# WhenMelancholy/ray-tracing-in-cuda

Measured on AMD Instinct MI355X. Metric: Msamples/sec (WxHxspp), higher is better.
Workload: dtype f32; 1 GPU; RTIOW random-spheres scene (rt_scene_rtiow seed 7, 484 spheres), 1920x1080, 1024 spp, depth 50; spp_chunk=0, kernel_variant=0, render_seed=2023

## Files before the change

### include/rtmi.h

```cpp
#ifndef RTMI_H
#define RTMI_H

#include <stddef.h>
#include <stdint.h>

#ifdef __cplusplus
extern "C" {
#endif

#define RTMI_ABI_VERSION 3

typedef enum rt_status {
    RT_OK = 0,
    RT_ERR_ARG = 1,
    RT_ERR_IO = 2,
    RT_ERR_JSON = 3,
    RT_ERR_SCENE = 4,
    RT_ERR_HIP = 5,
    RT_ERR_LIMIT = 6
} rt_status;


typedef enum rt_prim_type {
    RT_PRIM_SPHERE = 0,
// ... 269 lines not shown
int rt_scene_table_image(const rt_scene *s, float *out, int cap_floats);


typedef struct rt_opts {
    uint64_t seed;
    int32_t device;
    int32_t tile_rows;
    int32_t tile_first;
    int32_t tile_stride;
    int32_t tile_rotate;
    int32_t spp_chunk;
    int32_t sample_first;
    int32_t sample_count;
    uint32_t variant;
} rt_opts;

typedef struct rt_stats {
    double kernel_ms;
    double upload_ms;
    int32_t launches;
    int32_t local_rows;
    uint64_t samples, queries, prim_tests, hits, misses;
    uint64_t scatter[4];
    uint64_t rng_draws;
    uint64_t cand_lanes, cand_waves;
    uint64_t clusters_visited;
    uint64_t wave_queries;
    uint64_t groups_visited;
    uint64_t lane_clusters;
    uint64_t lane_groups;
// ... 158 lines not shown
```

### include/rtmi.hpp

```cpp
#pragma once
#include <cmath>
#include <memory>
#include <stdexcept>
#include <string>
#include <vector>

#include "rtmi.h"

namespace rtmi {

struct vec3 {
    float e[3];
    vec3() : e{0, 0, 0} {}
    vec3(float x, float y, float z) : e{x, y, z} {}
    float x() const { return e[0]; }
    float y() const { return e[1]; }
    float z() const { return e[2]; }
};
using point3 = vec3;
using color = vec3;

struct error : std::runtime_error {
    int status;
    error(int st, const std::string &where)
// ... 359 lines not shown
    void set_projection(rt_projection_type type, float p0 = 0.0f, float p1 = 0.0f) {
        const float p[2] = {p0, p1};
        check(rt_scene_set_projection(s_, type, type == RT_PROJ_PERSPECTIVE ? nullptr : p), "set_projection");
    }
    rt_projection_type projection(float params[2] = nullptr) const {
        int type = 0;
        check(rt_scene_get_projection(s_, &type, params), "projection");
        return (rt_projection_type)type;
    }
    bool camera_ray(float s, float t, rt_ray &out, float lx = 0.0f, float ly = 0.0f) const {
        int valid = 0;
        check(rt_camera_ray(s_, s, t, lx, ly, &out, &valid), "camera_ray");
        return valid != 0;
    }

    std::vector<rt_hit> trace(const std::vector<rt_ray> &rays, const rt_opts *opts = nullptr) const {
        std::vector<rt_hit> out(rays.size());
        check(rt_trace_hip(s_, opts, RT_TRACE_CLOSEST, rays.data(), rays.size(), out.data(), nullptr), "trace");
        return out;
    }
    std::vector<uint8_t> occluded(const std::vector<rt_ray> &rays, const rt_opts *opts = nullptr) const {
        std::vector<uint8_t> out(rays.size());
        check(rt_trace_hip(s_, opts, RT_TRACE_OCCLUDED, rays.data(), rays.size(), out.data(), nullptr), "occluded");
        return out;
    }

    rt_scene_info info() const {
        rt_scene_info i;
        check(rt_scene_get_info(s_, &i), "info");
        return i;
// ... 166 lines not shown
```

### ray-tracing-in-cuda_amd/__init__.py

```python
from __future__ import annotations

import ctypes as C
import os

import numpy as np

try:
    import torch
except Exception:
    torch = None

_HERE = os.path.dirname(os.path.abspath(__file__))
_LIB_PATH = os.environ.get("RTMI_LIB") or os.path.join(_HERE, "librtmi.so")
if not os.path.exists(_LIB_PATH):
    raise ImportError(
        f"{_LIB_PATH} not found: build it with `make -C {_HERE}` (or __graft_entry__.build()); "
        "this package has no fallback implementation"
    )
_lib = C.CDLL(_LIB_PATH)

RT_OK = 0
FLAG_SKY_GRADIENT = 1
FLAG_DEFOCUS_BLUR = 2
PRIM_SPHERE, PRIM_XY_RECT, PRIM_XZ_RECT, PRIM_YZ_RECT, PRIM_CYLINDER, PRIM_TRIANGLE, PRIM_QUAD = range(7)
# ... 267 lines not shown
_sig("rt_scene_clear_moving_spheres", C.c_int, _p)
_sig("rt_moving_sphere_hit", C.c_int, _p, C.c_float, _f3, _f3, C.c_float, C.POINTER(C.c_float))
_sig("rt_shutter_time", C.c_float, C.c_uint64, C.c_uint32, C.c_uint32)
_sig("rt_scene_add_point_light", C.c_int, _p, _f3, _f3)
_sig("rt_scene_add_spot_light", C.c_int, _p, _f3, _f3, _f3, C.c_float, C.c_float)
_sig("rt_scene_add_distant_light", C.c_int, _p, _f3, _f3, C.c_float)
_sig("rt_scene_get_analytic_lights", C.c_int, _p, _p, C.c_int)
_sig("rt_scene_clear_analytic_lights", C.c_int, _p)
assert _lib.rt_struct_size(25) == ANALYTIC_LIGHT_DTYPE.itemsize == 48
_sig("rt_scene_set_nested_grid", C.c_int, _p, C.c_int)
_sig("rt_scene_get_nested_grid", C.c_int, _p)
_sig("rt_scene_nested_info", C.c_int, _p, C.POINTER(NestedInfo))
_sig("rt_render_hip_count", C.c_int, _p, C.POINTER(Opts), _p, C.POINTER(Stats))
_sig("rt_scene_table_info", C.c_int, _p, C.POINTER(TableInfo))
_sig("rt_scene_table_image", C.c_int, _p, _p, C.c_int)
_sig("rt_render_hip_accumulate", C.c_int, _p, C.POINTER(Opts), _p, _p, C.POINTER(Stats))
_sig("rt_acc_to_rgb", None, _p, _p, C.c_size_t)
_sig("rt_render_hip_adaptive", C.c_int, _p, C.POINTER(Opts), C.POINTER(Adaptive), _p, _p, C.POINTER(AdaptiveStats))
_sig("rt_render_hip_adaptive_device", C.c_int, _p, C.POINTER(Opts), C.POINTER(Adaptive), _p, _p, _p, C.POINTER(AdaptiveStats))
_sig("rt_shard_scatter_rows", C.c_int, _p, C.POINTER(Opts), _p, _p)
_sig("rt_write_ppm", C.c_int, C.c_char_p, _p, C.c_int, C.c_int, C.c_int)
_sig("rt_quantize_rgb8", C.c_int, _p, C.c_int, C.c_int, C.c_int, C.c_int, _p)
_sig("rt_write_png", C.c_int, C.c_char_p, _p, C.c_int, C.c_int, C.c_int, C.c_int)
_sig("rt_scene_output_file", C.c_char_p, _p)
_sig("rt_philox4x32_10", None, C.POINTER(C.c_uint32), C.POINTER(C.c_uint32), C.POINTER(C.c_uint32))
_sig("rt_aabb_hit", C.c_int, _f3, _f3, _f3, _f3, C.c_float, C.c_float)
_sig("rt_sample_stream", None, C.c_uint64, C.c_uint32, C.c_uint32, C.POINTER(C.c_uint32), C.c_int)
_sig("rt_render_hip_feature", C.c_int, _p, C.POINTER(Opts), C.c_int, _p, C.POINTER(Stats))
_sig("rt_render_hip_feature_device", C.c_int, _p, C.POINTER(Opts), C.c_int, _p, _p, C.POINTER(Stats))
_sig("rt_trace_hip", C.c_int, _p, C.POINTER(Opts), C.c_int, _p, C.c_size_t, _p, C.POINTER(Stats))
# ... 7 lines not shown
     C.POINTER(C.c_double))
_sig("rt_denoise_hip_device", C.c_int, C.c_int, C.c_int, _p, C.c_int, _p, _p, _p, _p, C.c_int, C.POINTER(Denoise), C.c_int, _p, _p,
     C.POINTER(C.c_double))
_sig("rt_display_hip", C.c_int, C.c_int, C.c_int, _p, C.c_int, _p, C.POINTER(Display), C.c_int, _p, _p, C.POINTER(DisplayStats))
_sig("rt_display_hip_device", C.c_int, C.c_int, C.c_int, _p, C.c_int, _p, C.POINTER(Display), C.c_int, _p, _p, _p,
     C.POINTER(DisplayStats))
_sig("rt_display_timing", C.c_int, C.POINTER(C.c_double), C.c_int)
_sig("rt_write_ppm_rgb8", C.c_int, C.c_char_p, _p, C.c_int, C.c_int)
_sig("rt_write_png_rgb8", C.c_int, C.c_char_p, _p, C.c_int, C.c_int)
_sig("rt_write_hdr", C.c_int, C.c_char_p, _p, C.c_int, C.c_int, C.c_int)
_sig("rt_write_pfm", C.c_int, C.c_char_p, _p, C.c_int, C.c_int, C.c_int)

C_SYMBOLS = [
    "rt_last_error", "rt_status_string", "rt_abi_version", "rt_struct_size", "rt_device_count", "rt_has_ablations", "rt_opts_default",
    "rt_scene_table_info", "rt_scene_table_image", "rt_variant_workgroup",
    "rt_scene_load_json", "rt_scene_parse_json", "rt_scene_rtiow", "rt_scene_to_json", "rt_scene_free",
    "rt_scene_new", "rt_scene_set_background", "rt_scene_set_camera", "rt_scene_add_solid_color",
    "rt_scene_add_checker", "rt_scene_add_lambertian", "rt_scene_add_metal", "rt_scene_add_dielectric",
    "rt_scene_add_rough_metal", "rt_scene_add_plastic", "rt_scene_add_rough_glass", "rt_scene_add_noise_texture", "rt_scene_get_noise",
    "rt_scene_set_bump", "rt_scene_get_bump", "rt_scene_set_normal_map", "rt_scene_get_normal_map",
    "rt_scene_add_image_texture_rgba", "rt_scene_get_image_alpha", "rt_scene_set_alpha", "rt_scene_get_alpha", "rt_scene_add_pbr", "rt_scene_set_pbr_map", "rt_scene_get_pbr_map",
    "rt_scene_add_diffuse_light", "rt_scene_add_sphere", "rt_scene_add_rect", "rt_scene_add_cylinder",
    "rt_scene_add_image_texture", "rt_scene_add_image_texture_file", "rt_scene_get_image", "rt_scene_add_triangle",
    "rt_scene_add_quad", "rt_scene_add_box", "rt_scene_add_obj", "rt_scene_add_triangle_normals", "rt_scene_add_obj_normals", "rt_set_mesh_normals_override",
    "rt_scene_override", "rt_scene_get_info", "rt_scene_get_camera", "rt_scene_get_prims",
    "rt_scene_get_materials", "rt_scene_get_textures", "rt_shard_rows", "rt_shard_global_row", "rt_shard_deal",
    "rt_render_hip_device", "rt_render_hip", "rt_render_hip_tiles", "rt_tiles_shutdown", "rt_shard_place_rows_device", "rt_render_hip_count", "rt_render_hip_accumulate", "rt_scene_set_russian_roulette",
    "rt_acc_to_rgb", "rt_shard_scatter_rows", "rt_write_ppm",
    "rt_quantize_rgb8", "rt_philox4x32_10", "rt_aabb_hit", "rt_sample_stream", "rt_write_png",
    "rt_scene_output_file", "rt_scene_rotate_cylinders", "rt_scene_set_output_file", "rt_scene_dna", "rt_scene_clone",
# ... 544 lines not shown
                                         C.byref(stats) if stats is not None else None), "rt_render_hip_device")

    def table_info(self) -> TableInfo:
        t = TableInfo()
        _check(_lib.rt_scene_table_info(self._h, C.byref(t)), "rt_scene_table_info")
        return t

    def table_image(self) -> np.ndarray:
        n = _lib.rt_scene_table_image(self._h, None, 0)
        if n < 0:
            raise RtmiError(-n, "rt_scene_table_image")
        out = np.empty(n, dtype=np.float32)
        _lib.rt_scene_table_image(self._h, out.ctypes.data_as(C.c_void_p), n)
        return out.reshape(-1, 4)

    def count(self, opts: Opts | None = None, want_image=False):
        opts = opts or Opts()
        st = Stats()
        out = None
        ptr = None
        if want_image:
            out = np.empty((self.shard_rows(opts), self.width, 3), dtype=np.float32)
            ptr = out.ctypes.data_as(C.c_void_p)
        _check(_lib.rt_render_hip_count(self._h, C.byref(opts), ptr, C.byref(st)), "rt_render_hip_count")
        return (st, out) if want_image else st

    def accumulate(self, acc: np.ndarray | None = None, opts: Opts | None = None, stats: Stats | None = None,
                   want_image=True):
        opts = opts or Opts()
        rows = self.shard_rows(opts)
# ... 232 lines not shown
```

### ray-tracing-in-cuda_amd/csrc/device_scene.h

```cpp
#pragma once
#include <stdint.h>

#ifndef RTMI_ABLATIONS
#define RTMI_ABLATIONS 1
#endif

#define RT_CLUSTER 8
#define RT_MAX_SPHERE_SLOTS (1LL << 28)

#define RT_LIGHT_STRIDE 7

#define RT_CYL_STRIDE 6
#define RT_TRI_STRIDE 5
#define RT_QUAD_STRIDE 5
static_assert(RT_QUAD_STRIDE == RT_TRI_STRIDE, "quads and triangles share one hot table");

#ifndef RT_GROUP
#define RT_GROUP 4
#endif

#ifndef RT_SLABS
#define RT_SLABS 16
#endif

// ... 14 lines not shown
    MK_LIGHT_IMAGE = 7,
    MK_MEDIUM = 8,
    MK_ROUGH_METAL = 9,
    MK_PLASTIC_SOLID = 10,
    MK_PLASTIC_CHECKER = 11,
    MK_PLASTIC_IMAGE = 12,
    MK_LAMBERT_NOISE = 13,
    MK_LIGHT_NOISE = 14,
    MK_PLASTIC_NOISE = 15,
    MK_ROUGH_GLASS = 16,
    MK_PBR = 18
};

#define RT_ITEM_PARAMS_AT 16
#define RT_TILE_LIST_AT 64
struct ItemParams {
    int32_t tiles_x, bands, num_items, sample_first, sample_count, spp_chunk, n_big, n_med, q_med, q_small;
    int32_t tile_rows, tile_first, tile_stride, local_rows;
    int32_t tile_rotate;
    int32_t n_list = 0;
};

#define RT_PFLAG_NORMAL_MAPS (1u << 16)
#define RT_PFLAG_PROJ_SHIFT 17
#define RT_ALPHA_MAX_PASSES 64

struct RenderParams {
    int32_t off_cam;
    float background[3];
    uint32_t flags;
// ... 67 lines not shown
```

### ray-tracing-in-cuda_amd/csrc/kernels.h

```cpp
#pragma once
#include <hip/hip_runtime.h>
#include <stddef.h>

#include "device_scene.h"

namespace rtmi {

enum KernelFamily {
    K_PLAIN,
    K_NEE,
    K_NESTED,
    K_FEATURE,
    K_ENV,
    K_MEDIA,
    K_MOTION,
    K_TRACE,
};

struct KernelKey {
    KernelFamily family;
    unsigned variant;
    bool ext;
    bool count = false;
    bool nee = false;
// ... 1 lines not shown
    bool alpha = false;
    bool camera = false;
};

#ifndef RT_BIG_GROUPS
#define RT_BIG_GROUPS 1
#endif
#ifndef RT_BURSTS
#define RT_BURSTS 1
#endif
#ifndef RT_BURST_TRACE
#define RT_BURST_TRACE 1
#endif
#ifndef RT_BURST_REPOP
#define RT_BURST_REPOP 1
#endif
constexpr size_t kCuLdsBytes = 160 * 1024;
constexpr int kBurstIdBits = 15;
#ifndef RT_BIG_WAVES
#define RT_BIG_WAVES 15
#endif
#ifndef RT_BIG_WAVES_PER_SIMD
#define RT_BIG_WAVES_PER_SIMD 8
#endif
constexpr int kGroupWaves = 4, kBigGroupWaves = RT_BIG_WAVES;
constexpr int kBigGroupsPerCu = RT_BIG_WAVES_PER_SIMD / ((RT_BIG_WAVES + 3) / 4);
constexpr bool big_group(bool count, bool pool, bool scalar, int cull, bool sph) {
    return RT_BIG_GROUPS != 0 && sph && pool && !scalar && !count && (cull == 5 || cull == 6);
}
constexpr bool burst_starts(bool count, bool pool, bool scalar, int cull, bool sph) {
// ... 23 lines not shown
const KernelRow *camera_nee_kernel_rows(size_t *n);
const KernelRow *camera_media_kernel_rows(size_t *n);
const KernelRow *media_kernel_rows(size_t *n);
const KernelRow *motion_kernel_rows(size_t *n);
const KernelRow *trace_kernel_rows(size_t *n);

const KernelRow *find_kernel(const KernelKey &key);
void launch_kernel(const KernelRow &row, const RenderParams &P, const void *image, unsigned long long *acc, unsigned int *queue,
                   DevCounters *counters, size_t lds_bytes, unsigned grid, hipStream_t stream);
int blocks_per_cu(const KernelRow &row, size_t lds_bytes);
int set_max_dynamic_lds(const KernelRow &row, size_t bytes);
bool has_ablations();
void launch_finalize(const unsigned long long *acc, float *out, size_t n, hipStream_t stream);
void launch_item_params(unsigned int *queue, const ItemParams &ip, hipStream_t stream);

void launch_trace(const KernelRow &row, const RenderParams &P, const void *image, const void *rays, void *out, unsigned int *queue,
                  unsigned int n, int mode, size_t lds_bytes, unsigned grid, hipStream_t stream);

}
```

### ray-tracing-in-cuda_amd/csrc/render_body.h

```cpp
    extern __shared__ float4 lds[];
    constexpr bool GRID = CULL == 5 || CULL == 6 || CULL == 7 || CULL == 8, SHEET = CULL == 6, WIDE = CULL == 7 || CULL == 8;
    constexpr bool NEST = CULL == 8;
    static_assert(!NEST || (SCALAR && !SPH), "the nested walk reads its tables from global memory, in the general builds");
    constexpr int CSIZE = RT_CLUSTER;
    static_assert(!(CULL == 5 || CULL == 6) || SPH, "the compact grid tables list spheres only");
    static_assert(!(SPH && EXT), "image textures and triangles come with the general builds");
    static_assert(!QUERY || (EXT && POOL && !COUNT && !NEE && !AOV && !ENV && !MEDIA && !MOTION), "a ray query is the general build's walk and winner, nothing else");
    const int gap = (SCALAR || GRID) ? 0 : P.off_box - P.off_grid;
    const int staged = SCALAR ? 0 : (GRID ? P.hot_vec4_grid : (CULL == 3 ? P.hot_vec4_tables : P.hot_vec4) - gap);
    constexpr bool BIG = big_group(COUNT, POOL, SCALAR, CULL, SPH) && !QUERY && !NEE && !AOV && !ENV && !MEDIA && !MOTION;
    constexpr bool BURST = BIG && burst_starts(COUNT, POOL, SCALAR, CULL, SPH);
    constexpr bool TRACE = BURST && RT_BURST_TRACE != 0, REPOP = TRACE && RT_BURST_REPOP != 0;
    static_assert(kCuLdsBytes / 16 <= (size_t(1) << kBurstIdBits) && 16 + kBurstIdBits <= 31, "a staged sphere's id fits the bits above the row");
    constexpr int GW = BIG ? kBigGroupWaves : kGroupWaves;
    for (int i = threadIdx.x; i < staged; i += 64 * GW) lds[i] = image[i < P.off_grid ? i : i + gap];
    unsigned long long *tile_acc = reinterpret_cast<unsigned long long *>(lds + staged);
    if constexpr (!QUERY)
        for (int i = threadIdx.x; i < GW * 64 * 3; i += 64 * GW) tile_acc[i] = 0ull;
    __syncthreads();

    const int wave = __builtin_amdgcn_readfirstlane((int)(threadIdx.x >> 6)), lane = threadIdx.x & 63;
    unsigned long long *my_acc = tile_acc + wave * 192;
    float4 *slab_a = lds + staged + GW * (kWaveAccBytes / 16) + (BURST ? wave * (kWaveSlabBytes / 16) : 0);
    float4 *slab_b = slab_a + 64;
    float2 *slab_c = reinterpret_cast<float2 *>(slab_a + 128);
    const uint32_t k0 = P.seed_lo, k1 = P.seed_hi;
    const float4 *hot = SCALAR ? image : lds;
// ... 116 lines not shown
            }
        }
        tick(5);
        bool path_done = false;
        bool nee_add = false;
        float L_r = 0, L_g = 0, L_b = 0;
        asm volatile("" : "=v"(L_r), "=v"(L_g), "=v"(L_b));
        float px = 0, py = 0, pz = 0, nx = 0, ny = 0, nz = 0, inv_len = 0;
        int mat = 0, kind = -1;
        asm volatile("" : "=v"(px), "=v"(py), "=v"(pz), "=v"(nx), "=v"(ny), "=v"(nz), "=v"(inv_len), "=v"(mat));
        bool front = false;
        float tex_r = 0, tex_g = 0, tex_b = 0;
        if (VOTE_MASKS || __any(active)) {
        {
#define RT_QUERY_CUT true
#include "render_query.h"
#undef RT_QUERY_CUT
            if (active) {
#undef RT_SPHERE_TEST

            if (!SPH) {
                const bool any_far = GRID && (VOTE_MASKS ? far_m != 0ull : __builtin_amdgcn_ballot_w64(far_scan) != 0ull);
                const int nr_loop = (GRID && !any_far) ? P.nr_a : nr, nc_loop = (GRID && !any_far) ? P.nc_a : nc;
                const int nt_loop = EXT ? ((GRID && !any_far) ? P.nt_a : nt) : 0;
                for (int j = 0; j < nr_loop; ++j)
                    if (!GRID || j < P.nr_a || far_scan) test_rect(j);
                BoxP bq = {};
                const int nq_loop = EXT ? ((GRID && !any_far) ? P.nq_a : nq) : 0;
                if (CULL && (nc_loop > 0 || nt_loop > 0 || nq_loop > 0)) bq = box_params();
                for (int k = 0; k < nc_loop; ++k) {
                    const bool mine = !GRID || k < P.nc_a || far_scan;
// ... 1132 lines not shown
```

### ray-tracing-in-cuda_amd/csrc/render_burst.h

```cpp
                        float b_ox = 0.0f, b_oy = 0.0f, b_oz = 0.0f, b_dx = 0.0f, b_dy = 0.0f, b_dz = 1.0f;
                        bool b_live = false;
                        if (c_hy >= 0) {
                            const int bx = c_x0 + (lane & 7);
                            const int by = TRACE ? (c_hy & 0xffff) : c_hy;
                            const uint32_t pixel = __umul24((uint32_t)by, (uint32_t)P.width) + (uint32_t)bx;
                            LaneRng br;
                            br.draws = 0;
                            rng_start(br, pixel, (uint32_t)(c_sbegin + (cursor >> 6)), k0, k1);
                            const float bu = ((float)bx + rng_next<false>(br)) * P.inv_wm1;
                            const float bv = ((float)by + rng_next<false>(br)) * P.inv_hm1;
                            float offx = 0.0f, offy = 0.0f, offz = 0.0f;
                            const float4 *cv = hot + P.off_cam;
                            const float4 c_org = cv[0];
                            if (P.flags & RT_FLAG_DEFOCUS_BLUR) {
                                float bsx, bsy;
                                do {
                                    bsx = rng_pm1<false>(br);
                                    bsy = rng_pm1<false>(br);
                                } while (fmaf(bsx, bsx, bsy * bsy) >= 1.0f);
                                const float4 c_u = cv[4], c_v = cv[5];
                                const float rdx = c_org.w * bsx, rdy = c_org.w * bsy;
                                offx = fmaf(c_u.x, rdx, c_v.x * rdy);
                                offy = fmaf(c_u.y, rdx, c_v.y * rdy);
                                offz = fmaf(c_u.z, rdx, c_v.z * rdy);
// ... 12 lines not shown
                                }
                                b_ox = c_org.x + offx, b_oy = c_org.y + offy, b_oz = c_org.z + offz;
                                b_dx = bdx, b_dy = bdy, b_dz = bdz;
                            } else {
                                slab_a[lane] = make_float4(c_org.x + offx, c_org.y + offy, c_org.z + offz, bdx);
                            }
                            slab_b[lane] = make_float4(bdy, bdz, __uint_as_float(br.g.x), __uint_as_float(br.g.y));
                            slab_c[lane] = make_float2(__uint_as_float(br.g.z), __uint_as_float(br.g.w));
                        } else {
                            if constexpr (!TRACE) slab_a[lane] = make_float4(0.0f, 0.0f, 0.0f, __uint_as_float(0x7fc00000u));
                        }
                        if constexpr (TRACE) {
                            const float ox = b_ox, oy = b_oy, oz = b_oz, dx = b_dx, dy = b_dy, dz = b_dz;
                            const float ra = dot3(dx, dy, dz, dx, dy, dz), rinv_a = 1.0f / ra;
                            const bool active = b_live;
                            float t_res = 0.0f;
                            float4 rec = make_float4(0.0f, 0.0f, 0.0f, __uint_as_float(0x7fc00000u));
                            {
#define RT_QUERY_CUT false
#include "render_query.h"
#undef RT_QUERY_CUT
#undef RT_SPHERE_TEST
                                if (active) {
                                    const float bb = P.rr_p > 0.0f ? 1.0f / P.rr_p : 1.0f;
                                    float e_r = 0.0f, e_g = 0.0f, e_b = 0.0f;
                                    bool ends = true;
                                    if (best_id >= 0) {
                                        const float4 cold = *rec_at(image + P.off_sph_cold, (uint32_t)best_id << 4);
                                        const float hx = fmaf(best_t, dx, ox), hy = fmaf(best_t, dy, oy), hz = fmaf(best_t, dz, oz);
                                        const int hkind = __float_as_int(cold.w);
                                        if (hkind >= MK_LIGHT_SOLID && (!EXT || hkind <= MK_LIGHT_IMAGE)) {
                                            const float4 *M = image + P.off_mat + 3 * __float_as_int(cold.y);
                                            const float4 q1 = M[1], q2 = M[2];
                                            const bool odd = hkind == MK_LIGHT_CHECKER && checker_odd(hx, hy, hz);
                                            e_r = (odd ? q2.x : q1.x) * bb, e_g = (odd ? q2.y : q1.y) * bb, e_b = (odd ? q2.z : q1.z) * bb;
                                        } else {
// ... 28 lines not shown
```

### ray-tracing-in-cuda_amd/csrc/render_host.hip

```cpp
#include <hip/hip_runtime.h>

#include <algorithm>
#include <array>
#include <cmath>
#include <cstdint>
#include <cstdlib>
#include <cstring>
#include <memory>
#include <mutex>
#include <vector>

#include "device_scene.h"
#include "hip_host.h"
#include "kernels.h"
#include "pack.h"
#include "scene.hpp"
#include "shard.h"

namespace rtmi {

void launch_adaptive_estimate(const long long *A, const long long *B, const unsigned int *list, int n_list, unsigned int *next_list,
                              unsigned int *next_count, int *tile_n, int width, int height, int tiles_x, int nA, int nB, int n,
                              bool retire_all, bool use_metric, double t4, hipStream_t stream);
void launch_adaptive_merge(const long long *A, const long long *B, const int *tile_n, float *out, int *spp_map, int width, int height,
                           int tiles_x, hipStream_t stream);
static const KernelRow *variant_row(unsigned variant, bool ext = false, bool count = false, bool alpha = false, bool camera = false) {
    const KernelRow *row = find_kernel({K_PLAIN, variant, ext, count, false, false, alpha, camera});
    return row ? row : find_kernel({K_NESTED, variant, ext, count, false, false, alpha, camera});
}

static bool variant_exists(unsigned variant) { return variant == 0 || variant_row(variant); }

struct DeviceEntry {
    int device = -1;
    uint64_t version = 0;
    DeviceBuffer<float> d_image;
    DeviceBuffer<unsigned long long> d_acc;
    DeviceBuffer<DevCounters> d_counters;
    DeviceBuffer<float> d_out;
    DeviceBuffer<char> d_adapt;
    DeviceBuffer<int> d_spp;
    DeviceBuffer<unsigned int> d_trace_queue;
    DeviceBuffer<char> d_trace_io;
    int num_cus = 0;
};

struct DeviceSceneCache {
    std::mutex mu;
    std::vector<std::unique_ptr<DeviceEntry>> entries;
    uint64_t packed_version = 0;
    std::vector<float> image;
    RenderParams layout;
    NestedInfo nested;
};

static DeviceSceneCache &cache_of(const Scene &s) {
    Scene &ms = const_cast<Scene &>(s);
    if (!ms.dev) ms.dev = std::make_shared<DeviceSceneCache>();
    return *ms.dev;
}

static int ensure_packed(const Scene &s, DeviceSceneCache &cache) {
    if (cache.packed_version == s.version) return RT_OK;
    std::vector<float> image;
    RenderParams layout;
    NestedInfo nested;
    int rc = pack_scene(s, image, layout, &nested);
    if (rc) return rc;
    cache.image = std::move(image);
    cache.layout = layout;
    cache.nested = nested;
    cache.packed_version = s.version;
    return RT_OK;
}

struct Shard {
    int tile_rows, tile_first, tile_stride, tile_rotate, num_tiles, local_tiles, local_rows;
};

static int shard_of(const Scene &s, const rt_opts *o, Shard &sh) {
    sh.tile_rows = (o && o->tile_rows > 0) ? o->tile_rows : 8;
    sh.tile_first = o ? o->tile_first : 0;
    sh.tile_stride = (o && o->tile_stride > 1) ? o->tile_stride : 1;
    sh.tile_rotate = (o && sh.tile_stride > 1) ? o->tile_rotate : 0;
    if (sh.tile_rotate < 0 || sh.tile_rotate > 2) {
        set_error("tile_rotate %d: 0 (plain interleave), 1 (rotated) or 2 (there and back)", sh.tile_rotate);
        return RT_ERR_ARG;
// ... 150 lines not shown
        return RT_ERR_ARG;
    }
    int rc = scene_validate(sc->s);
    if (rc) return rc;
    DeviceSceneCache &cache = cache_of(sc->s);
    std::lock_guard<std::mutex> lock(cache.mu);
    rc = ensure_packed(sc->s, cache);
    if (rc) return rc;
    const NestedInfo &n = cache.nested;
    memset(out, 0, sizeof *out);
    out->cells = n.cells, out->sub_cells = n.sub_cells, out->sub_items = n.sub_items;
    out->off_sub_grids = n.off_sub_grids, out->off_sub_cells = n.off_sub_cells, out->first_sub_cell = n.first_sub_cell;
    out->threshold = n.threshold, out->axis_cap = n.axis_cap, out->longest = n.longest;
    return RT_OK;
}

int rt_scene_table_image(const rt_scene *sc, float *dst, int cap_floats) {
    rt_table_info info;
    int rc = read_tables(sc, &info, dst, cap_floats);
    return rc ? -rc : info.image_floats;
}

struct ChunkPlan {
    int spp_chunk, num_chunks, n_big, n_med, q_med, q_small, orphan_max;
};

static ChunkPlan plan_chunks(long long tiles, int sample_count, int spp_chunk_opt) {
    int spp_chunk = spp_chunk_opt > 0 ? spp_chunk_opt : 0;
    if (spp_chunk == 0) {
        const long long want_items = 8LL * 256 * RT_WAVES_PER_SIMD * 4;
// ... 39 lines not shown
    int max_spp;
    int *d_spp_map;
    rt_adaptive_stats *st;
};

struct Launcher {
    const RenderParams &P;
    const Shard &sh;
    DeviceEntry *ent;
    DevCounters *d_cnt;
    hipStream_t stream;
    size_t lds_bytes;
    unsigned long long resident;
    const KernelRow &kernel;
    int feature;

    int enqueue(unsigned long long *acc, unsigned int *d_queue, int first, int n, int n_list, const ChunkPlan &pl) const {
        RenderParams Q = P;
        Q.sample_first = first, Q.sample_count = n;
        Q.spp_chunk = pl.spp_chunk, Q.num_chunks = pl.num_chunks;
        Q.n_big = pl.n_big, Q.n_med = pl.n_med, Q.q_med = pl.q_med, Q.q_small = pl.q_small;
        Q.orphan_max = pl.orphan_max;
        const unsigned long long items = (unsigned long long)(n_list ? n_list : (long long)P.tiles_x * P.bands) * pl.num_chunks;
        if (items > 0x7fffffffull) {
            set_error("%llu work items exceed the queue counter", items);
            return RT_ERR_LIMIT;
        }
        Q.num_items = (int)items;
        {
            ItemParams ip;
            ip.tiles_x = n_list ? n_list : Q.tiles_x, ip.bands = n_list ? 1 : Q.bands, ip.num_items = Q.num_items;
            ip.sample_first = Q.sample_first, ip.sample_count = Q.sample_count, ip.spp_chunk = Q.spp_chunk;
            ip.n_big = Q.n_big, ip.n_med = Q.n_med, ip.q_med = Q.q_med, ip.q_small = Q.q_small;
            ip.tile_rows = Q.tile_rows, ip.tile_first = Q.tile_first, ip.tile_stride = Q.tile_stride;
            ip.tile_rotate = sh.tile_rotate;
            ip.local_rows = Q.local_rows;
            ip.n_list = n_list;
            launch_item_params(d_queue, ip, stream);
        }
        const unsigned long long need_blocks = (items + kernel.waves - 1) / kernel.waves;
        const unsigned long long grid = need_blocks < resident ? (need_blocks ? need_blocks : 1) : resident;
        if (feature >= 0) Q.feature = feature;
        launch_kernel(kernel, Q, ent->d_image.get(), acc, d_queue, d_cnt, lds_bytes, (unsigned)grid, stream);
        return RT_OK;
    }
};

static int run_adaptive(const Launcher &launch, const AdaptiveRun &ad, const Scene &s, size_t queue_off, size_t need, float *d_out,
                        int spp_chunk_opt, int &launches) {
    const RenderParams &P = launch.P;
    DeviceEntry *ent = launch.ent;
    const hipStream_t stream = launch.stream;
    const long long frame_tiles = (long long)P.tiles_x * P.bands;
// ... 470 lines not shown
    DevCounters *d_cnt = nullptr;
    if (count) {
        rc = ent->d_counters.reserve(1);
        if (rc) return rc;
        d_cnt = ent->d_counters.get();
        HIP_TRY(hipMemsetAsync(d_cnt, 0, sizeof(DevCounters), stream));
        HIP_TRY(hipMemsetAsync(&d_cnt->t_start_min, 0xff, sizeof(unsigned long long), stream));
        HIP_TRY(hipMemsetAsync(&d_cnt->t_end_min, 0xff, sizeof(unsigned long long), stream));
        HIP_TRY(hipMemsetAsync(&d_cnt->t_qe_min, 0xff, sizeof(unsigned long long), stream));
    }
    if (stats) HIP_TRY(hipEventRecord(ev1, stream));

    const size_t queue_off = (plane * sizeof(unsigned long long) + 255) & ~(size_t)255;
    const long long frame_tiles = (long long)P.tiles_x * P.bands;
    const size_t need = queue_off + (ad ? (((size_t)(RT_TILE_LIST_AT + frame_tiles) * 4 + 255) & ~(size_t)255) : 256);
    const Launcher launch{P, sh, ent, d_cnt, stream, lds_bytes, resident, *kernel, feature};

    int launches = 0;
    if (ad) {
        rc = run_adaptive(launch, *ad, s, queue_off, need, d_out, o ? o->spp_chunk : 0, launches);
        if (rc) return rc;
    } else if (s.max_depth <= 0 && !h_acc && feature < 0) {
        HIP_TRY(hipMemsetAsync(d_out, 0, plane * sizeof(float), stream));
    } else {
        rc = ent->d_acc.reserve(need / sizeof(unsigned long long));
        if (rc) return rc;
        unsigned long long *const d_acc = ent->d_acc.get();
        HIP_TRY(hipMemsetAsync(d_acc, 0, need, stream));
        if (h_acc) HIP_TRY(hipMemcpyAsync(d_acc, h_acc, plane * sizeof(long long), hipMemcpyHostToDevice, stream));
        unsigned int *d_queue = reinterpret_cast<unsigned int *>(reinterpret_cast<char *>(d_acc) + queue_off);
        if (s.max_depth > 0 || feature >= 0) {
// ... 367 lines not shown
```

### ray-tracing-in-cuda_amd/csrc/render_query.h

```cpp
            float best_t = QUERY ? q_tmax : (NEE && shadow != 0 && !(ENV && (shadow & 4) != 0)) ? 0.999f : INFINITY;
            if constexpr (ALPHA && NEE) {
                if (shadow != 0 && !(ENV && (shadow & 4) != 0)) best_t = 0.999f - al_state[AL_T];
            }
            int best_id = -1;

            auto resolve = [&](int idx, float hb, float disc) {
                if (COUNT) {
                    c_cand++;
                    const unsigned long long em = __builtin_amdgcn_ballot_w64(true);
                    if ((int)__builtin_ctzll(em) == lane) c_cand_wave++;
                }
                const float sq = rt_sqrtf<ROOT_VOTE>(disc);
                float root = (-hb - sq) * rinv_a;
                if (root < kTMin || best_t < root) root = (-hb + sq) * rinv_a;
                bool take = !(root < kTMin || best_t < root);
                const bool tie = take && root == best_t && best_id >= 0;
                if (__builtin_expect(__builtin_amdgcn_ballot_w64(tie) != 0ull, 0)) {
                    if (tie) take = lidx(idx) > lidx(best_id);
                }
                best_t = take ? root : best_t;
                best_id = take ? idx : best_id;
            };
            float tq_a = 1.0f, tq_ux = 0.0f, tq_uy = 0.0f, tq_uz = 0.0f;
            if (EXT && nt > 0 && active) {
// ... 23 lines not shown
        if (__builtin_expect(cand, 0)) resolve(IDX, hb, disc);                                 \
    }
#define RT_SPHERE_PARK(S, IDX)                                                                 \
    {                                                                                          \
        const float ocx = ox - S.x, ocy = oy - S.y, ocz = oz - S.z;                            \
        const float hb = dot3(ocx, ocy, ocz, dx, dy, dz);                                      \
        const float cc = fmaf(ocx, ocx, fmaf(ocy, ocy, fmaf(ocz, ocz, -S.w)));                 \
        const float disc = fmaf(hb, hb, -(ra * cc));                                           \
        const bool cand = RT_CAND(disc, hb, cc);                                                \
        if (__builtin_expect(cand, 0)) {                                                       \
            if (p_idx >= 0) resolve(p_idx, p_hb, p_disc);                                      \
            p_idx = IDX, p_hb = hb, p_disc = disc;                                             \
        }                                                                                      \
    }
            if (RT_PRIO_Q != RT_PRIO_S) __builtin_amdgcn_s_setprio(RT_PRIO_Q);
            if (active) {
            for (int i = 0; i < P.np; i += 4) {
                const float4 s0 = sph[i], s1 = sph[i + 1], s2 = sph[i + 2], s3 = sph[i + 3];
                RT_SPHERE_TEST(s0, i)
                int p_idx = -1;
                float p_hb = 0.0f, p_disc = 0.0f;
                asm volatile("" : "=v"(p_hb), "=v"(p_disc));
                RT_SPHERE_PARK(s1, i + 1)
                RT_SPHERE_PARK(s2, i + 2)
                RT_SPHERE_PARK(s3, i + 3)
                if (p_idx >= 0) resolve(p_idx, p_hb, p_disc);
            }
            if (!CULL) {
                {
                    constexpr int kStep = 2 * (CSIZE + 1);
#define RT_OFF(k) ((k) + ((k) >= CSIZE ? 1 : 0))
// ... 160 lines not shown
                    float t, qa, qb;
                    if (quad_hit(r0.x, r0.y, r0.z, r0.w, r1.w, r2.w, r1.x, r1.y, r1.z, r2.x, r2.y, r2.z, ox, oy, oz, dx, dy, dz, kTMin,
                                 best_t, t, qa, qb)) {
                        bool take = true;
                        if (t == best_t && best_id >= 0)
                            take = list_index_of(P, image, ns + nr + nc + nt + k) > list_index_of(P, image, best_id);
                        if (take) {
                            best_t = t;
                            best_id = ns + nr + nc + nt + k;
                        }
                    }
                }
            };
            bool far_scan = false;
            unsigned long long far_m = 0ull;
            if (active) {
            if (GRID && P.grid_cells != 0) {
                const float4 *gh = hot + P.off_grid;
                const float4 g_min = gh[0], g_inv = gh[1], g_size = gh[2];
                const int gnx = __float_as_int(gh[3].x), gny = __float_as_int(gh[3].y), gnz = __float_as_int(gh[3].z);
                const uint32_t *g_cells = reinterpret_cast<const uint32_t *>(hot + P.off_grid_cells);
                const uint16_t *g_items = reinterpret_cast<const uint16_t *>(hot + P.off_grid_items);
                const BoxP bp = box_params();
                const float o2 = fmaf(ox, ox, fmaf(oy, oy, oz * oz));
                const bool tier_far = o2 > g_min.w, beyond = o2 > g_inv.w;
                const int cnt_shift = tier_far ? (WIDE ? 10 : 0) : (WIDE ? 0 : 6);
                constexpr int REM_BITS = WIDE ? 10 : 8;
                constexpr uint32_t REM_MASK = (1u << REM_BITS) - 1u, CNT_MASK = WIDE ? 1023u : 63u;
                constexpr bool OTHERS = WIDE && !SPH;
                const uint32_t *g_items32 = reinterpret_cast<const uint32_t *>(g_items);
                int ko = 0, koend = 0;
// ... 381 lines not shown
```

Measured before the change: 22040 Msamples/s.

## Add per-tile camera beam sphere lists to skip full scans for primary rays

Builds a per-8x8-tile table on the GPU listing up to 15 sphere slots that a conservative beam from the camera through each tile can reach, with an overflow marker otherwise. Burst-traced rays in these kernels read the tile's record and, when it is listed, test only those spheres instead of running the full sphere, cluster and grid query. The table is cached per scene version and camera, and its address is passed through the queue. This aims to cut intersection work for camera rays, at the cost of an extra table build, a scalar table load per burst, and reliance on a conservative double-precision bound being correct.

```diff
diff --git a/include/rtmi.h b/include/rtmi.h
--- a/include/rtmi.h
+++ b/include/rtmi.h
@@ -307,6 +307,9 @@
     int32_t sample_count;
     uint32_t variant;
 } rt_opts;
+int rt_scene_tile_beams(const rt_scene *s, uint16_t *out, int cap_tiles);
+int rt_scene_tile_beams_device(const rt_scene *s, const rt_opts *o, uint16_t *out, int cap_tiles);
+int rt_scene_tile_beams_capacity(void);
 
 typedef struct rt_stats {
     double kernel_ms;
diff --git a/include/rtmi.hpp b/include/rtmi.hpp
--- a/include/rtmi.hpp
+++ b/include/rtmi.hpp
@@ -397,6 +397,15 @@
         return valid != 0;
     }
 
+    std::vector<uint16_t> tile_beams(bool on_device = false, const rt_opts *opts = nullptr) const {
+        const int n = on_device ? rt_scene_tile_beams_device(s_, opts, nullptr, 0) : rt_scene_tile_beams(s_, nullptr, 0);
+        check(n < 0 ? -n : 0, "tile_beams");
+        std::vector<uint16_t> out((size_t)n * 16);
+        const int m = on_device ? rt_scene_tile_beams_device(s_, opts, out.data(), n) : rt_scene_tile_beams(s_, out.data(), n);
+        check(m < 0 ? -m : 0, "tile_beams");
+        return out;
+    }
+
     std::vector<rt_hit> trace(const std::vector<rt_ray> &rays, const rt_opts *opts = nullptr) const {
         std::vector<rt_hit> out(rays.size());
         check(rt_trace_hip(s_, opts, RT_TRACE_CLOSEST, rays.data(), rays.size(), out.data(), nullptr), "trace");
diff --git a/ray-tracing-in-cuda_amd/__init__.py b/ray-tracing-in-cuda_amd/__init__.py
--- a/ray-tracing-in-cuda_amd/__init__.py
+++ b/ray-tracing-in-cuda_amd/__init__.py
@@ -305,6 +305,9 @@
 _sig("rt_render_hip_count", C.c_int, _p, C.POINTER(Opts), _p, C.POINTER(Stats))
 _sig("rt_scene_table_info", C.c_int, _p, C.POINTER(TableInfo))
 _sig("rt_scene_table_image", C.c_int, _p, _p, C.c_int)
+_sig("rt_scene_tile_beams", C.c_int, _p, _p, C.c_int)
+_sig("rt_scene_tile_beams_device", C.c_int, _p, C.POINTER(Opts), _p, C.c_int)
+_sig("rt_scene_tile_beams_capacity", C.c_int)
 _sig("rt_render_hip_accumulate", C.c_int, _p, C.POINTER(Opts), _p, _p, C.POINTER(Stats))
 _sig("rt_acc_to_rgb", None, _p, _p, C.c_size_t)
 _sig("rt_render_hip_adaptive", C.c_int, _p, C.POINTER(Opts), C.POINTER(Adaptive), _p, _p, C.POINTER(AdaptiveStats))
@@ -342,6 +345,7 @@
 C_SYMBOLS = [
     "rt_last_error", "rt_status_string", "rt_abi_version", "rt_struct_size", "rt_device_count", "rt_has_ablations", "rt_opts_default",
     "rt_scene_table_info", "rt_scene_table_image", "rt_variant_workgroup",
+    "rt_scene_tile_beams", "rt_scene_tile_beams_device", "rt_scene_tile_beams_capacity",
     "rt_scene_load_json", "rt_scene_parse_json", "rt_scene_rtiow", "rt_scene_to_json", "rt_scene_free",
     "rt_scene_new", "rt_scene_set_background", "rt_scene_set_camera", "rt_scene_add_solid_color",
     "rt_scene_add_checker", "rt_scene_add_lambertian", "rt_scene_add_metal", "rt_scene_add_dielectric",
@@ -916,6 +920,26 @@
         _lib.rt_scene_table_image(self._h, out.ctypes.data_as(C.c_void_p), n)
         return out.reshape(-1, 4)
 
+    def tile_beams(self, opts: Opts | None = None, device=False) -> np.ndarray:
+        name = "rt_scene_tile_beams_device" if device else "rt_scene_tile_beams"
+        call = (lambda p, n: _lib.rt_scene_tile_beams_device(self._h, C.byref(opts) if opts is not None else None, p, n)) if device else \
+               (lambda p, n: _lib.rt_scene_tile_beams(self._h, p, n))
+        n = call(None, 0)
+        if n < 0:
+            raise RtmiError(-n, name)
+        out = np.empty((n, 16), dtype=np.uint16)
+        n = call(out.ctypes.data_as(C.c_void_p), n)
+        if n < 0:
+            raise RtmiError(-n, name)
+        info = self.info
+        return out.reshape((int(info.height) + 7) // 8, (int(info.width) + 7) // 8, 16)
+
+    def tile_beam_list(self, tx: int, ty: int):
+        rec = self.tile_beams()[ty, tx]
+        if rec[0] == 0xffff:
+            return [], True
+        return [int(i) for i in rec[1:1 + int(rec[0])]], False
+
     def count(self, opts: Opts | None = None, want_image=False):
         opts = opts or Opts()
         st = Stats()
diff --git a/ray-tracing-in-cuda_amd/csrc/device_scene.h b/ray-tracing-in-cuda_amd/csrc/device_scene.h
--- a/ray-tracing-in-cuda_amd/csrc/device_scene.h
+++ b/ray-tracing-in-cuda_amd/csrc/device_scene.h
@@ -52,6 +52,7 @@
 
 #define RT_ITEM_PARAMS_AT 16
 #define RT_TILE_LIST_AT 64
+#define RT_BEAMS_AT 32
 struct ItemParams {
     int32_t tiles_x, bands, num_items, sample_first, sample_count, spp_chunk, n_big, n_med, q_med, q_small;
     int32_t tile_rows, tile_first, tile_stride, local_rows;
diff --git a/ray-tracing-in-cuda_amd/csrc/kernels.h b/ray-tracing-in-cuda_amd/csrc/kernels.h
--- a/ray-tracing-in-cuda_amd/csrc/kernels.h
+++ b/ray-tracing-in-cuda_amd/csrc/kernels.h
@@ -3,6 +3,7 @@
 #include <stddef.h>
 
 #include "device_scene.h"
+#include "rt_beam.h"
 
 namespace rtmi {
 
@@ -39,6 +40,9 @@
 #endif
 #ifndef RT_BURST_REPOP
 #define RT_BURST_REPOP 1
+#endif
+#ifndef RT_BURST_LISTS
+#define RT_BURST_LISTS 1
 #endif
 constexpr size_t kCuLdsBytes = 160 * 1024;
 constexpr int kBurstIdBits = 15;
@@ -92,6 +96,9 @@
 void launch_finalize(const unsigned long long *acc, float *out, size_t n, hipStream_t stream);
 void launch_item_params(unsigned int *queue, const ItemParams &ip, hipStream_t stream);
 
+void launch_tile_beams(const float *image, const BeamFrame &f, int tiles_x, int tiles_y, uint16_t *table, hipStream_t stream);
+void launch_beam_address(unsigned int *queue, const uint16_t *table, hipStream_t stream);
+
 void launch_trace(const KernelRow &row, const RenderParams &P, const void *image, const void *rays, void *out, unsigned int *queue,
                   unsigned int n, int mode, size_t lds_bytes, unsigned grid, hipStream_t stream);
 
diff --git a/ray-tracing-in-cuda_amd/csrc/render_body.h b/ray-tracing-in-cuda_amd/csrc/render_body.h
--- a/ray-tracing-in-cuda_amd/csrc/render_body.h
+++ b/ray-tracing-in-cuda_amd/csrc/render_body.h
@@ -11,6 +11,7 @@
     constexpr bool BIG = big_group(COUNT, POOL, SCALAR, CULL, SPH) && !QUERY && !NEE && !AOV && !ENV && !MEDIA && !MOTION;
     constexpr bool BURST = BIG && burst_starts(COUNT, POOL, SCALAR, CULL, SPH);
     constexpr bool TRACE = BURST && RT_BURST_TRACE != 0, REPOP = TRACE && RT_BURST_REPOP != 0;
+    constexpr bool LISTS = TRACE && RT_BURST_LISTS != 0;
     static_assert(kCuLdsBytes / 16 <= (size_t(1) << kBurstIdBits) && 16 + kBurstIdBits <= 31, "a staged sphere's id fits the bits above the row");
     constexpr int GW = BIG ? kBigGroupWaves : kGroupWaves;
     for (int i = threadIdx.x; i < staged; i += 64 * GW) lds[i] = image[i < P.off_grid ? i : i + gap];
@@ -157,7 +158,9 @@
         if (VOTE_MASKS || __any(active)) {
         {
 #define RT_QUERY_CUT true
+#define RT_QUERY_SKIP false
 #include "render_query.h"
+#undef RT_QUERY_SKIP
 #undef RT_QUERY_CUT
             if (active) {
 #undef RT_SPHERE_TEST
diff --git a/ray-tracing-in-cuda_amd/csrc/render_burst.h b/ray-tracing-in-cuda_amd/csrc/render_burst.h
--- a/ray-tracing-in-cuda_amd/csrc/render_burst.h
+++ b/ray-tracing-in-cuda_amd/csrc/render_burst.h
@@ -1,5 +1,17 @@
                         float b_ox = 0.0f, b_oy = 0.0f, b_oz = 0.0f, b_dx = 0.0f, b_dy = 0.0f, b_dz = 1.0f;
                         bool b_live = false;
+                        [[maybe_unused]] unsigned long long b_w0 = kBeamOverflow, b_w1 = 0ull, b_w2 = 0ull, b_w3 = 0ull;
+                        if constexpr (LISTS) {
+                            typedef const __attribute__((address_space(4))) unsigned long long *BeamWords;
+                            asm volatile("" ::: "memory");
+                            const unsigned long long b_table = *(BeamWords)(uintptr_t)(queue + RT_BEAMS_AT);
+                            if (b_table != 0ull) {
+                                const int b_ty = (__builtin_amdgcn_readfirstlane(c_hy) & 0xffff) >> 3;
+                                const uint32_t b_tile = __umul24((uint32_t)b_ty, (uint32_t)P.tiles_x) + (uint32_t)(c_x0 >> 3);
+                                BeamWords b_rec = (BeamWords)(uintptr_t)(b_table + (unsigned long long)b_tile * (kBeamRecordWords * 2));
+                                b_w0 = b_rec[0], b_w1 = b_rec[1], b_w2 = b_rec[2], b_w3 = b_rec[3];
+                            }
+                        }
                         if (c_hy >= 0) {
                             const int bx = c_x0 + (lane & 7);
                             const int by = TRACE ? (c_hy & 0xffff) : c_hy;
@@ -50,12 +62,26 @@
                             const float ox = b_ox, oy = b_oy, oz = b_oz, dx = b_dx, dy = b_dy, dz = b_dz;
                             const float ra = dot3(dx, dy, dz, dx, dy, dz), rinv_a = 1.0f / ra;
                             const bool active = b_live;
+                            [[maybe_unused]] const bool b_listed = LISTS && (uint32_t)(b_w0 & 0xffffull) != (uint32_t)kBeamOverflow;
                             float t_res = 0.0f;
                             float4 rec = make_float4(0.0f, 0.0f, 0.0f, __uint_as_float(0x7fc00000u));
                             {
 #define RT_QUERY_CUT false
+#define RT_QUERY_SKIP (LISTS && b_listed)
 #include "render_query.h"
+#undef RT_QUERY_SKIP
 #undef RT_QUERY_CUT
+                                if constexpr (LISTS) {
+                                    if (b_listed) {
+                                        for (int b_n = (int)(b_w0 & 0xffffull); b_n > 0; --b_n) {
+                                            b_w0 = (b_w0 >> 16) | (b_w1 << 48), b_w1 = (b_w1 >> 16) | (b_w2 << 48);
+                                            b_w2 = (b_w2 >> 16) | (b_w3 << 48), b_w3 >>= 16;
+                                            const int b_id = (int)(b_w0 & 0xffffull);
+                                            const float4 b_s = sph[b_id];
+                                            if (active) RT_SPHERE_TEST(b_s, b_id)
+                                        }
+                                    }
+                                }
 #undef RT_SPHERE_TEST
                                 if (active) {
                                     const float bb = P.rr_p > 0.0f ? 1.0f / P.rr_p : 1.0f;
diff --git a/ray-tracing-in-cuda_amd/csrc/render_host.hip b/ray-tracing-in-cuda_amd/csrc/render_host.hip
--- a/ray-tracing-in-cuda_amd/csrc/render_host.hip
+++ b/ray-tracing-in-cuda_amd/csrc/render_host.hip
@@ -30,6 +30,18 @@
 }
 
 static bool variant_exists(unsigned variant) { return variant == 0 || variant_row(variant); }
+
+struct BeamKey {
+    bool valid = false;
+    uint64_t version = 0;
+    const void *image = nullptr;
+    BeamFrame frame{};
+    float camera[16] = {};
+    bool same(const BeamKey &o) const {
+        return valid && o.valid && version == o.version && image == o.image && !memcmp(&frame, &o.frame, sizeof frame) &&
+               !memcmp(camera, o.camera, sizeof camera);
+    }
+};
 
 struct DeviceEntry {
     int device = -1;
@@ -42,6 +54,8 @@
     DeviceBuffer<int> d_spp;
     DeviceBuffer<unsigned int> d_trace_queue;
     DeviceBuffer<char> d_trace_io;
+    DeviceBuffer<uint16_t> d_beams;
+    BeamKey beams_key;
     int num_cus = 0;
 };
 
@@ -71,6 +85,37 @@
     cache.layout = layout;
     cache.nested = nested;
     cache.packed_version = s.version;
+    return RT_OK;
+}
+
+static BeamFrame beam_frame_of(const Scene &s, const RenderParams &L) {
+    BeamFrame f;
+    memset(&f, 0, sizeof f);
+    f.off_cam = L.off_cam, f.nslots = L.np + (RT_CLUSTER + 1) * L.ncl;
+    f.width = s.width, f.height = s.height;
+    f.inv_wm1 = 1.0f / (float)(s.width - 1), f.inv_hm1 = 1.0f / (float)(s.height - 1);
+    f.defocus = (s.flags & RT_FLAG_DEFOCUS_BLUR) ? 1u : 0u;
+    return f;
+}
+
+static bool beams_apply(const Scene &s, const RenderParams &L) {
+    return !L.grid_wide && s.cam.projection == RT_PROJ_PERSPECTIVE && s.width > 1 && s.height > 1 &&
+           L.np + (RT_CLUSTER + 1) * L.ncl <= 65535;
+}
+
+static int ensure_beams(const Scene &s, const DeviceSceneCache &cache, DeviceEntry *ent, hipStream_t stream) {
+    BeamKey key;
+    key.valid = true, key.version = ent->version, key.image = ent->d_image.get();
+    key.frame = beam_frame_of(s, cache.layout);
+    memcpy(key.camera, cache.image.data() + 4 * (size_t)cache.layout.off_cam, sizeof key.camera);
+    const int tiles_x = (s.width + 7) / 8, tiles_y = (s.height + 7) / 8;
+    if (ent->beams_key.same(key) && ent->d_beams.get()) return RT_OK;
+    ent->beams_key.valid = false;
+    int rc = ent->d_beams.reserve((size_t)tiles_x * tiles_y * kBeamRecordWords);
+    if (rc) return rc;
+    launch_tile_beams(ent->d_image.get(), key.frame, tiles_x, tiles_y, ent->d_beams.get(), stream);
+    HIP_TRY(hipGetLastError());
+    ent->beams_key = key;
     return RT_OK;
 }
 
@@ -251,6 +296,73 @@
     out->threshold = n.threshold, out->axis_cap = n.axis_cap, out->longest = n.longest;
     return RT_OK;
 }
+
+int rt_scene_tile_beams(const rt_scene *sc, uint16_t *out, int cap_tiles) {
+    if (!sc) {
+        set_error("rt_scene_tile_beams: null scene");
+        return -RT_ERR_ARG;
+    }
+    int rc = scene_validate(sc->s);
+    if (rc) return -rc;
+    const Scene &s = sc->s;
+    DeviceSceneCache &cache = cache_of(s);
+    std::lock_guard<std::mutex> lock(cache.mu);
+    rc = ensure_packed(s, cache);
+    if (rc) return -rc;
+    if (!beams_apply(s, cache.layout)) {
+        set_error("rt_scene_tile_beams: the bursts of this scene read no lists (compact sphere tables, the perspective camera and a frame of at least 2 x 2 pixels have them)");
+        return -RT_ERR_LIMIT;
+    }
+    const int tiles_x = (s.width + 7) / 8, tiles_y = (s.height + 7) / 8;
+    const BeamFrame f = beam_frame_of(s, cache.layout);
+    for (int t = 0; out && t < tiles_x * tiles_y && t < cap_tiles; ++t)
+        beam_tile_record(cache.image.data(), f, t % tiles_x, t / tiles_x, out + (size_t)t * kBeamRecordWords);
+    return tiles_x * tiles_y;
+}
+
+int rt_scene_tile_beams_device(const rt_scene *sc, const rt_opts *o, uint16_t *out, int cap_tiles) {
+    if (!sc) {
+        set_error("rt_scene_tile_beams_device: null scene");
+        return -RT_ERR_ARG;
+    }
+    int rc = scene_validate(sc->s);
+    if (rc) return -rc;
+    const Scene &s = sc->s;
+    const int device = o ? o->device : 0;
+    DeviceScope scope;
+    rc = scope.enter(device, "the beam table");
+    if (rc) return -rc;
+    DeviceSceneCache &cache = cache_of(s);
+    std::lock_guard<std::mutex> lock(cache.mu);
+    rc = ensure_packed(s, cache);
+    if (rc) return -rc;
+    if (!beams_apply(s, cache.layout)) {
+        set_error("rt_scene_tile_beams_device: the bursts of this scene read no lists (compact sphere tables, the perspective camera and a frame of at least 2 x 2 pixels have them)");
+        return -RT_ERR_LIMIT;
+    }
+    DeviceEntry *ent = device_record(cache.entries, device);
+    if (ent->version != s.version || !ent->d_image.get()) {
+        rc = ent->d_image.reserve(cache.image.size());
+        if (rc) return -rc;
+        if (hipMemcpy(ent->d_image.get(), cache.image.data(), cache.image.size() * sizeof(float), hipMemcpyHostToDevice) != hipSuccess) {
+            set_error("rt_scene_tile_beams_device: the upload of the scene image failed");
+            return -RT_ERR_HIP;
+        }
+        ent->version = s.version;
+    }
+    rc = ensure_beams(s, cache, ent, nullptr);
+    if (rc) return -rc;
+    const int tiles = ((s.width + 7) / 8) * ((s.height + 7) / 8);
+    const int n = std::min(tiles, cap_tiles);
+    if (hipStreamSynchronize(nullptr) != hipSuccess ||
+        (out && n > 0 && hipMemcpy(out, ent->d_beams.get(), (size_t)n * kBeamRecordWords * sizeof(uint16_t), hipMemcpyDeviceToHost) != hipSuccess)) {
+        set_error("rt_scene_tile_beams_device: reading the table back failed");
+        return -RT_ERR_HIP;
+    }
+    return tiles;
+}
+
+int rt_scene_tile_beams_capacity(void) { return kBeamCapacity; }
 
 int rt_scene_table_image(const rt_scene *sc, float *dst, int cap_floats) {
     rt_table_info info;
@@ -320,6 +432,7 @@
     unsigned long long resident;
     const KernelRow &kernel;
     int feature;
+    const uint16_t *beams;
 
     int enqueue(unsigned long long *acc, unsigned int *d_queue, int first, int n, int n_list, const ChunkPlan &pl) const {
         RenderParams Q = P;
@@ -343,6 +456,7 @@
             ip.local_rows = Q.local_rows;
             ip.n_list = n_list;
             launch_item_params(d_queue, ip, stream);
+            if (beams) launch_beam_address(d_queue, beams, stream);
         }
         const unsigned long long need_blocks = (items + kernel.waves - 1) / kernel.waves;
         const unsigned long long grid = need_blocks < resident ? (need_blocks ? need_blocks : 1) : resident;
@@ -843,7 +957,14 @@
     const size_t queue_off = (plane * sizeof(unsigned long long) + 255) & ~(size_t)255;
     const long long frame_tiles = (long long)P.tiles_x * P.bands;
     const size_t need = queue_off + (ad ? (((size_t)(RT_TILE_LIST_AT + frame_tiles) * 4 + 255) & ~(size_t)255) : 256);
-    const Launcher launch{P, sh, ent, d_cnt, stream, lds_bytes, resident, *kernel, feature};
+    const uint16_t *beams = nullptr;
+    if (RT_BURST_LISTS != 0 && kernel->key.family == K_PLAIN && !kernel->key.count && (kernel->cull == 5 || kernel->cull == 6) &&
+        sh.tile_rows % 8 == 0 && beams_apply(s, cache.layout)) {
+        rc = ensure_beams(s, cache, ent, stream);
+        if (rc) return rc;
+        beams = ent->d_beams.get();
+    }
+    const Launcher launch{P, sh, ent, d_cnt, stream, lds_bytes, resident, *kernel, feature, beams};
 
     int launches = 0;
     if (ad) {
diff --git a/ray-tracing-in-cuda_amd/csrc/render_query.h b/ray-tracing-in-cuda_amd/csrc/render_query.h
--- a/ray-tracing-in-cuda_amd/csrc/render_query.h
+++ b/ray-tracing-in-cuda_amd/csrc/render_query.h
@@ -61,7 +61,7 @@
         }                                                                                      \
     }
             if (RT_PRIO_Q != RT_PRIO_S) __builtin_amdgcn_s_setprio(RT_PRIO_Q);
-            if (active) {
+            if (active && !RT_QUERY_SKIP) {
             for (int i = 0; i < P.np; i += 4) {
                 const float4 s0 = sph[i], s1 = sph[i + 1], s2 = sph[i + 2], s3 = sph[i + 3];
                 RT_SPHERE_TEST(s0, i)
@@ -252,7 +252,7 @@
             };
             bool far_scan = false;
             unsigned long long far_m = 0ull;
-            if (active) {
+            if (active && !RT_QUERY_SKIP) {
             if (GRID && P.grid_cells != 0) {
                 const float4 *gh = hot + P.off_grid;
                 const float4 g_min = gh[0], g_inv = gh[1], g_size = gh[2];
diff --git a/ray-tracing-in-cuda_amd/csrc/rt_beam.h b/ray-tracing-in-cuda_amd/csrc/rt_beam.h
--- /dev/null
+++ b/ray-tracing-in-cuda_amd/csrc/rt_beam.h
@@ -0,0 +1,97 @@
+#pragma once
+#include <math.h>
+#include <stdint.h>
+
+#ifdef __HIPCC__
+#define RTMI_BEAM_HD __host__ __device__ inline
+#else
+#define RTMI_BEAM_HD inline
+#endif
+
+namespace rtmi {
+
+constexpr int kBeamRecordWords = 16;
+constexpr int kBeamCapacity = kBeamRecordWords - 1;
+constexpr uint16_t kBeamOverflow = 0xffffu;
+
+struct BeamFrame {
+    int32_t off_cam;
+    int32_t nslots;
+    int32_t width, height;
+    float inv_wm1, inv_hm1;
+    uint32_t defocus;
+};
+
+struct Beam {
+    double ax, ay, az, dx, dy, dz, dd;
+    double lens, rho, m;
+};
+
+RTMI_BEAM_HD Beam beam_of_tile(const float *image, const BeamFrame &f, int tx, int ty) {
+    const float *cv = image + 4 * (size_t)f.off_cam;
+    const double iw = (double)f.inv_wm1, ih = (double)f.inv_hm1;
+    const double uc = (double)(8 * tx + 4) * iw, vc = (double)(8 * ty + 4) * ih;
+    Beam b;
+    b.ax = cv[0], b.ay = cv[1], b.az = cv[2];
+    b.lens = f.defocus ? fabs((double)cv[3]) : 0.0;
+    const double hx = cv[8], hy = cv[9], hz = cv[10], vx = cv[12], vy = cv[13], vz = cv[14];
+    b.dx = ((double)cv[4] + uc * hx + vc * vx) - b.ax;
+    b.dy = ((double)cv[5] + uc * hy + vc * vy) - b.ay;
+    b.dz = ((double)cv[6] + uc * hz + vc * vz) - b.az;
+    b.dd = b.dx * b.dx + b.dy * b.dy + b.dz * b.dz;
+    const double px = 4.0 * iw * hx, py = 4.0 * iw * hy, pz = 4.0 * iw * hz;
+    const double qx = 4.0 * ih * vx, qy = 4.0 * ih * vy, qz = 4.0 * ih * vz;
+    b.rho = sqrt((px * px + py * py + pz * pz) + (qx * qx + qy * qy + qz * qz) + 2.0 * fabs(px * qx + py * qy + pz * qz));
+    double n1 = b.lens;
+    for (int i = 0; i < 16; ++i)
+        if ((i & 3) != 3) n1 += fabs((double)cv[i]);
+    b.m = 64.0 * 5.9604644775390625e-08 * n1;
+    return b;
+}
+
+RTMI_BEAM_HD bool beam_quad_reaches(double a, double b, double c, double lo, double hi) {
+    if ((a * lo + 2.0 * b) * lo + c <= 0.0) return true;
+    if (hi >= 0.0 && (a * hi + 2.0 * b) * hi + c <= 0.0) return true;
+    if (a > 0.0) {
+        const double tv = -b / a;
+        return tv > lo && (hi < 0.0 || tv < hi) && (a * tv + 2.0 * b) * tv + c <= 0.0;
+    }
+    return hi < 0.0;
+}
+
+RTMI_BEAM_HD bool beam_reaches(const Beam &b, double cx, double cy, double cz, double r2) {
+    const double wx = b.ax - cx, wy = b.ay - cy, wz = b.az - cz;
+    const double ww = wx * wx + wy * wy + wz * wz, wd = wx * b.dx + wy * b.dy + wz * b.dz;
+    const double reach = sqrt(ww) + b.lens;
+    const double rp = sqrt(r2 + (32.0 * 5.9604644775390625e-08) * (reach * reach));
+    {
+        const double al = rp + b.lens + b.m, be = b.rho - b.lens + b.m;
+        if (beam_quad_reaches(b.dd - be * be, wd - al * be, ww - al * al, 0.0, 1.0)) return true;
+    }
+    {
+        const double al = rp - b.lens + b.m, be = b.rho + b.lens + b.m;
+        if (beam_quad_reaches(b.dd - be * be, wd - al * be, ww - al * al, 1.0, -1.0)) return true;
+    }
+    return false;
+}
+
+RTMI_BEAM_HD void beam_tile_record(const float *image, const BeamFrame &f, int tx, int ty, uint16_t *rec) {
+    const Beam b = beam_of_tile(image, f, tx, ty);
+    int n = 0;
+    for (int k = 1; k < kBeamRecordWords; ++k) rec[k] = 0;
+    for (int i = 0; i < f.nslots; ++i) {
+        const float *s = image + 4 * (size_t)i;
+        if (!(s[3] >= 0.0f)) continue;
+        if (!beam_reaches(b, (double)s[0], (double)s[1], (double)s[2], (double)s[3])) continue;
+        if (n < kBeamCapacity) rec[1 + n] = (uint16_t)i;
+        ++n;
+    }
+    if (n > kBeamCapacity) {
+        for (int k = 1; k < kBeamRecordWords; ++k) rec[k] = 0;
+        rec[0] = kBeamOverflow;
+    } else {
+        rec[0] = (uint16_t)n;
+    }
+}
+
+}
diff --git a/ray-tracing-in-cuda_amd/csrc/tile_beams.hip b/ray-tracing-in-cuda_amd/csrc/tile_beams.hip
--- /dev/null
+++ b/ray-tracing-in-cuda_amd/csrc/tile_beams.hip
@@ -0,0 +1,47 @@
+#include <hip/hip_runtime.h>
+
+#include "kernels.h"
+
+namespace rtmi {
+
+__global__ void __launch_bounds__(64) tile_beams_kernel(const float *image, BeamFrame f, int tiles_x, uint16_t *table) {
+    __shared__ uint16_t rec[kBeamRecordWords];
+    const int t = (int)blockIdx.x, lane = (int)threadIdx.x;
+    const int ty = t / tiles_x, tx = t - ty * tiles_x;
+    const Beam b = beam_of_tile(image, f, tx, ty);
+    if (lane < kBeamRecordWords) rec[lane] = 0;
+    __syncthreads();
+    int n = 0;
+    for (int base = 0; base < f.nslots; base += 64) {
+        const int i = base + lane;
+        bool reached = false;
+        if (i < f.nslots) {
+            const float4 s = reinterpret_cast<const float4 *>(image)[i];
+            reached = s.w >= 0.0f && beam_reaches(b, (double)s.x, (double)s.y, (double)s.z, (double)s.w);
+        }
+        const unsigned long long m = __ballot(reached);
+        const int at = n + __popcll(m & ((1ull << lane) - 1ull));
+        if (reached && at < kBeamCapacity) rec[1 + at] = (uint16_t)i;
+        n += __popcll(m);
+    }
+    __syncthreads();
+    if (lane < kBeamRecordWords) {
+        const uint16_t w = lane == 0 ? (n > kBeamCapacity ? kBeamOverflow : (uint16_t)n) : (n > kBeamCapacity ? (uint16_t)0 : rec[lane]);
+        table[(size_t)t * kBeamRecordWords + lane] = w;
+    }
+}
+
+__global__ void beam_address_kernel(unsigned int *queue, unsigned long long address) {
+    queue[RT_BEAMS_AT] = (unsigned int)address;
+    queue[RT_BEAMS_AT + 1] = (unsigned int)(address >> 32);
+}
+
+void launch_tile_beams(const float *image, const BeamFrame &f, int tiles_x, int tiles_y, uint16_t *table, hipStream_t stream) {
+    hipLaunchKernelGGL(tile_beams_kernel, dim3((unsigned)(tiles_x * tiles_y)), dim3(64), 0, stream, image, f, tiles_x, table);
+}
+
+void launch_beam_address(unsigned int *queue, const uint16_t *table, hipStream_t stream) {
+    hipLaunchKernelGGL(beam_address_kernel, dim3(1), dim3(1), 0, stream, queue, (unsigned long long)(uintptr_t)table);
+}
+
+}
```

Measured after the change: 23100 Msamples/s (median of 6 runs). 4.8% higher.
